# VisionDepth/VisionDepth3D

Hardware: NVIDIA H100
Metric: end-to-end frames/sec (depth+stereo) (higher is better)
Workload: dtype f16 GEMM operands, fp32 accumulate; DIBR fp32

## Files before the change

visiondepth3d_b200/csrc/umma_gemm.cuh:

```cuda
#pragma once
#include <cuda.h>
#include <cuda_fp16.h>
#include <cuda_runtime.h>
#include <stdint.h>

namespace vd3d {

enum Epi : int {
  EPI_F16 = 0,
  EPI_F32 = 1,
  EPI_RESID_LS = 2,
  EPI_QKV = 3,
  EPI_PATCH = 4,
  EPI_CONVT = 5,
  EPI_HEAD = 6,
  EPI_SR = 7,
  EPI_READOUT = 8,
};

struct GemmArgs {
  int M, N, K;
  int nt, mt, nz;
  int epi;
  int act;
  int conv;
  int cin;
  int imgW, imgH;
  int tw, th;
  __half* out_f16;
  __half* out2_f16;
  const __half* res_f16;
  float* out_f32;
  const float* bias;
  const float* ls;
  const float* pos;
  int ldc;
  long long out_batch_stride;
  __half* q;
  __half* k;
  __half* vt;
  int heads, npad, dmodel;
  float qscale;
  int ct_k, ct_cout, ct_w;
  const float* w3;
  const float* b3p;
  const __half* res2_f16;
  float rs, rs2;
  const float* img_bias;
};

namespace umma {

__device__ __forceinline__ uint32_t smem_u32(const void* p) { return (uint32_t)__cvta_generic_to_shared(p); }

__device__ __forceinline__ void mbar_init(uint32_t bar, uint32_t count) {
  asm volatile("mbarrier.init.shared::cta.b64 [%0], %1;" ::"r"(bar), "r"(count));
}
__device__ __forceinline__ void mbar_expect_tx(uint32_t bar, uint32_t bytes) {
  asm volatile("mbarrier.arrive.expect_tx.shared::cta.b64 _, [%0], %1;" ::"r"(bar), "r"(bytes) : "memory");
}
__device__ __forceinline__ void mbar_arrive(uint32_t bar) {
  asm volatile("mbarrier.arrive.shared::cta.b64 _, [%0];" ::"r"(bar) : "memory");
}
__device__ __forceinline__ void mbar_wait(uint32_t bar, uint32_t parity) {
  asm volatile(
      "{\n"
      ".reg .pred P1;\n"
      "LAB_WAIT:\n"
      "mbarrier.try_wait.parity.shared::cta.b64 P1, [%0], %1;\n"
      "@P1 bra DONE;\n"
      "bra LAB_WAIT;\n"
      "DONE:\n"
      "}\n" ::"r"(bar),
      "r"(parity)
      : "memory");
}
__device__ __forceinline__ void fence_barrier_init() {
  asm volatile("fence.mbarrier_init.release.cluster;" ::: "memory");
}

__device__ __forceinline__ void tma_load_3d(uint32_t dst, const CUtensorMap* tm, uint32_t bar, int c0, int c1,
                                            int c2) {
  asm volatile(
      "cp.async.bulk.tensor.3d.shared::cluster.global.mbarrier::complete_tx::bytes [%0], [%1, {%3, %4, %5}], [%2];"
      ::"r"(dst), "l"((uint64_t)tm), "r"(bar), "r"(c0), "r"(c1), "r"(c2)
      : "memory");
}
__device__ __forceinline__ void prefetch_tmap(const CUtensorMap* tm) {
  asm volatile("prefetch.tensormap [%0];" ::"l"((uint64_t)tm) : "memory");
}

__device__ __forceinline__ uint64_t make_desc(uint32_t smem_addr) {
  uint64_t d = 0;
  d |= (uint64_t)((smem_addr >> 4) & 0x3FFF);
  d |= (uint64_t)1 << 16;
  d |= (uint64_t)(1024 >> 4) << 32;
  d |= (uint64_t)1 << 62;
  return d;
}

__device__ __forceinline__ void wgmma_fence() { asm volatile("wgmma.fence.sync.aligned;" ::: "memory"); }
__device__ __forceinline__ void wgmma_commit() { asm volatile("wgmma.commit_group.sync.aligned;" ::: "memory"); }
template <int N>
__device__ __forceinline__ void wgmma_wait() {
  asm volatile("wgmma.wait_group.sync.aligned %0;" ::"n"(N) : "memory");
}
template <int R>
__device__ __forceinline__ void fence_regs(float (&d)[R]) {
#pragma unroll
  for (int i = 0; i < R; ++i) asm volatile("" : "+f"(d[i])::"memory");
}

#define VD3D_ACC8(i) "+f"(d[i]), "+f"(d[i + 1]), "+f"(d[i + 2]), "+f"(d[i + 3]), "+f"(d[i + 4]), "+f"(d[i + 5]), \
                     "+f"(d[i + 6]), "+f"(d[i + 7])
__device__ __forceinline__ void wgmma_m64n32_ss(float (&d)[16], uint64_t da, uint64_t db, uint32_t accumulate) {
  asm volatile(
      "{\n"
      ".reg .pred p;\n"
      "setp.ne.b32 p, %18, 0;\n"
      "wgmma.mma_async.sync.aligned.m64n32k16.f32.f16.f16 "
      "{%0, %1, %2, %3, %4, %5, %6, %7, %8, %9, %10, %11, %12, %13, %14, %15}, "
      "%16, %17, p, 1, 1, 0, 0;\n"
      "}\n"
      : VD3D_ACC8(0), VD3D_ACC8(8)
      : "l"(da), "l"(db), "r"(accumulate));
}
__device__ __forceinline__ void wgmma_m64n64_ss(float (&d)[32], uint64_t da, uint64_t db, uint32_t accumulate) {
  asm volatile(
      "{\n"
      ".reg .pred p;\n"
      "setp.ne.b32 p, %34, 0;\n"
      "wgmma.mma_async.sync.aligned.m64n64k16.f32.f16.f16 "
      "{%0, %1, %2, %3, %4, %5, %6, %7, %8, %9, %10, %11, %12, %13, %14, %15, %16, %17, %18, %19, %20, %21, %22, %23, %24, %25, %26, %27, %28, %29, %30, %31}, "
      "%32, %33, p, 1, 1, 0, 0;\n"
      "}\n"
      : VD3D_ACC8(0), VD3D_ACC8(8), VD3D_ACC8(16), VD3D_ACC8(24)
      : "l"(da), "l"(db), "r"(accumulate));
}
__device__ __forceinline__ void wgmma_m64n128_ss(float (&d)[64], uint64_t da, uint64_t db, uint32_t accumulate) {
  asm volatile(
      "{\n"
      ".reg .pred p;\n"
      "setp.ne.b32 p, %66, 0;\n"
      "wgmma.mma_async.sync.aligned.m64n128k16.f32.f16.f16 "
      "{%0, %1, %2, %3, %4, %5, %6, %7, %8, %9, %10, %11, %12, %13, %14, %15, %16, %17, %18, %19, %20, %21, %22, %23, %24, %25, %26, %27, %28, %29, %30, %31, %32, %33, %34, %35, %36, %37, %38, %39, %40, %41, %42, %43, %44, %45, %46, %47, %48, %49, %50, %51, %52, %53, %54, %55, %56, %57, %58, %59, %60, %61, %62, %63}, "
      "%64, %65, p, 1, 1, 0, 0;\n"
      "}\n"
      : VD3D_ACC8(0), VD3D_ACC8(8), VD3D_ACC8(16), VD3D_ACC8(24), VD3D_ACC8(32), VD3D_ACC8(40), VD3D_ACC8(48), VD3D_ACC8(56)
      : "l"(da), "l"(db), "r"(accumulate));
}
__device__ __forceinline__ void wgmma_m64n64_rs(float (&d)[32], const uint32_t (&a)[4], uint64_t db, uint32_t accumulate) {
  asm volatile(
      "{\n"
      ".reg .pred p;\n"
      "setp.ne.b32 p, %37, 0;\n"
      "wgmma.mma_async.sync.aligned.m64n64k16.f32.f16.f16 "
      "{%0, %1, %2, %3, %4, %5, %6, %7, %8, %9, %10, %11, %12, %13, %14, %15, %16, %17, %18, %19, %20, %21, %22, %23, %24, %25, %26, %27, %28, %29, %30, %31}, "
      "{%32, %33, %34, %35}, %36, p, 1, 1, 0;\n"
      "}\n"
      : VD3D_ACC8(0), VD3D_ACC8(8), VD3D_ACC8(16), VD3D_ACC8(24)
      : "r"(a[0]), "r"(a[1]), "r"(a[2]), "r"(a[3]), "l"(db), "r"(accumulate));
}

template <int N>
__device__ __forceinline__ void wgmma_ss(float (&d)[N / 2], uint64_t da, uint64_t db, uint32_t accumulate) {
  if constexpr (N == 32) wgmma_m64n32_ss(d, da, db, accumulate);
  else if constexpr (N == 64) wgmma_m64n64_ss(d, da, db, accumulate);
  else wgmma_m64n128_ss(d, da, db, accumulate);
}

__device__ __forceinline__ float ex2_fast(float x) {
  float y;
  asm("ex2.approx.ftz.f32 %0, %1;" : "=f"(y) : "f"(x));
  return y;
}

__device__ __forceinline__ float gelu_erf(float x) {
  const float ax = fabsf(x);
  const float z = ax * 0.70710678118654752440f;
  float t;
  asm("rcp.approx.ftz.f32 %0, %1;" : "=f"(t) : "f"(fmaf(0.3275911f, z, 1.0f)));
  float p = fmaf(t, 1.061405429f, -1.453152027f);
  p = fmaf(t, p, 1.421413741f);
  p = fmaf(t, p, -0.284496736f);
  p = fmaf(t, p, 0.254829592f);
  p *= t;
  const float e = ex2_fast(x * x * -0.72134752044448170368f);
  return fmaf(-0.5f * ax * p, e, fmaxf(x, 0.f));
}

__device__ __forceinline__ void ldg_v8(const void* p, uint32_t (&r)[8]) {
  asm volatile("ld.global.v4.b32 {%0, %1, %2, %3}, [%8];\n\t"
               "ld.global.v4.b32 {%4, %5, %6, %7}, [%8+16];"
               : "=r"(r[0]), "=r"(r[1]), "=r"(r[2]), "=r"(r[3]), "=r"(r[4]), "=r"(r[5]), "=r"(r[6]), "=r"(r[7])
               : "l"(p));
}
__device__ __forceinline__ void ldg_nc_v8(const void* p, uint32_t (&r)[8]) {
  asm volatile("ld.global.nc.v4.b32 {%0, %1, %2, %3}, [%8];\n\t"
               "ld.global.nc.v4.b32 {%4, %5, %6, %7}, [%8+16];"
               : "=r"(r[0]), "=r"(r[1]), "=r"(r[2]), "=r"(r[3]), "=r"(r[4]), "=r"(r[5]), "=r"(r[6]), "=r"(r[7])
               : "l"(p));
}
__device__ __forceinline__ void stg_v8(void* p, const uint32_t (&r)[8]) {
  asm volatile("st.global.v4.b32 [%0], {%1, %2, %3, %4};\n\t"
               "st.global.v4.b32 [%0+16], {%5, %6, %7, %8};" ::"l"(p), "r"(r[0]), "r"(r[1]), "r"(r[2]),
               "r"(r[3]), "r"(r[4]), "r"(r[5]), "r"(r[6]), "r"(r[7])
               : "memory");
}
__device__ __forceinline__ void pack16(const float (&a)[32], int base, bool relu, uint32_t (&u)[8]) {
#pragma unroll
  for (int t = 0; t < 8; ++t) {
    float x = a[base + 2 * t], y = a[base + 2 * t + 1];
    if (relu) {
      x = fmaxf(x, 0.f);
      y = fmaxf(y, 0.f);
    }
    __half2 h = __floats2half2_rn(x, y);
    u[t] = *(uint32_t*)&h;
  }
}

}

__device__ __forceinline__ void sr_epilogue_chunk(const GemmArgs& g, float (&a)[32], const int m, const int n0,
                                                  const int nvalid, const bool full) {
  if (g.out_f32) {
    float* dst = g.out_f32 + (size_t)m * g.ldc + n0;
    if (full && ((((size_t)m * g.ldc + n0) & 3) == 0)) {
#pragma unroll
      for (int j = 0; j < 8; ++j) ((float4*)dst)[j] = make_float4(a[4 * j], a[4 * j + 1], a[4 * j + 2], a[4 * j + 3]);
    } else {
#pragma unroll
      for (int j = 0; j < 32; ++j)
        if (j < nvalid) dst[j] = a[j];
    }
    return;
  }
  size_t o;
  if (g.ct_k) {
    const int tap = n0 / g.ct_cout, co = n0 % g.ct_cout;
    const int dy = tap / g.ct_k, dx = tap % g.ct_k;
    const int y = m / g.ct_w, x = m % g.ct_w;
    o = ((size_t)(y * g.ct_k + dy) * (g.ct_w * g.ct_k) + (x * g.ct_k + dx)) * g.ct_cout + co;
  } else {
    o = (size_t)m * g.ldc + n0;
  }
  const bool vec = full && ((o & 15) == 0);
#pragma unroll
  for (int q = 0; q < 2; ++q) {
    const __half* res = q == 0 ? g.res_f16 : g.res2_f16;
    if (!res) continue;
    const float sc = q == 0 ? g.rs : g.rs2;
    float rv[32];
    if (vec) {
      uint32_t u[2][8];
      umma::ldg_v8(res + o, u[0]);
      umma::ldg_v8(res + o + 16, u[1]);
#pragma unroll
      for (int j = 0; j < 2; ++j)
#pragma unroll
        for (int t = 0; t < 8; ++t) {
          const float2 f = __half22float2(*(const __half2*)&u[j][t]);
          rv[16 * j + 2 * t] = f.x;
          rv[16 * j + 2 * t + 1] = f.y;
        }
    } else {
#pragma unroll
      for (int j = 0; j < 32; ++j) rv[j] = (j < nvalid) ? __half2float(res[o + j]) : 0.f;
    }
#pragma unroll
    for (int j = 0; j < 32; ++j) a[j] = rv[j] + sc * a[j];
  }
  if (g.act == 4) {
#pragma unroll
    for (int j = 0; j < 32; ++j) a[j] = a[j] > 0.f ? a[j] : 0.2f * a[j];
  }
  if (vec) {
    uint32_t u[8];
    umma::pack16(a, 0, false, u);
    umma::stg_v8(g.out_f16 + o, u);
    umma::pack16(a, 16, false, u);
    umma::stg_v8(g.out_f16 + o + 16, u);
  } else {
#pragma unroll
    for (int j = 0; j < 32; ++j)
      if (j < nvalid) g.out_f16[o + j] = __float2half_rn(a[j]);
  }
}

template <bool kSr>
__device__ __forceinline__ void gemm_epilogue_chunk(const GemmArgs& g, const uint32_t (&v)[32], const int m, const int z,
                                                    const int n0, const bool row_ok, float& head_acc) {
  if (!row_ok || n0 >= g.N) return;
  const int nvalid = min(32, g.N - n0);
  const bool full = (nvalid == 32);
  float a[32];
  if (g.bias) {
    if (full) {
#pragma unroll
      for (int j = 0; j < 8; ++j) {
        float4 b4 = __ldg((const float4*)(g.bias + n0) + j);
        a[4 * j + 0] = __uint_as_float(v[4 * j + 0]) + b4.x;
        a[4 * j + 1] = __uint_as_float(v[4 * j + 1]) + b4.y;
        a[4 * j + 2] = __uint_as_float(v[4 * j + 2]) + b4.z;
        a[4 * j + 3] = __uint_as_float(v[4 * j + 3]) + b4.w;
      }
    } else {
#pragma unroll
      for (int j = 0; j < 32; ++j) a[j] = __uint_as_float(v[j]) + ((j < nvalid) ? g.bias[n0 + j] : 0.f);
    }
  } else {
#pragma unroll
    for (int j = 0; j < 32; ++j) a[j] = __uint_as_float(v[j]);
  }
  if constexpr (kSr) {
    sr_epilogue_chunk(g, a, m, n0, nvalid, full);
    return;
  }
  switch (g.epi) {
    case EPI_F16: {
      const size_t o = (size_t)z * g.out_batch_stride + (size_t)m * g.ldc + n0;
      const bool vec = full && ((o & 15) == 0);
      if (g.res_f16) {
        if (vec) {
          uint32_t rv[2][8];
          umma::ldg_nc_v8(g.res_f16 + o, rv[0]);
          umma::ldg_nc_v8(g.res_f16 + o + 16, rv[1]);
#pragma unroll
          for (int j = 0; j < 2; ++j)
#pragma unroll
            for (int t = 0; t < 8; ++t) {
              float2 f = __half22float2(*(const __half2*)&rv[j][t]);
              a[16 * j + 2 * t] += f.x;
              a[16 * j + 2 * t + 1] += f.y;
            }
        } else {
#pragma unroll
          for (int j = 0; j < 32; ++j)
            if (j < nvalid) a[j] += __half2float(g.res_f16[o + j]);
        }
      }
      if (g.act == 1) {
#pragma unroll
        for (int j = 0; j < 32; ++j) a[j] = umma::gelu_erf(a[j]);
      } else if (g.act == 2) {
#pragma unroll
        for (int j = 0; j < 32; ++j) a[j] = fmaxf(a[j], 0.f);
      } else if (g.act == 3) {
#pragma unroll
        for (int j = 0; j < 32; ++j)
          if (j < nvalid) a[j] = a[j] > 0.f ? a[j] : a[j] * __ldg(g.ls + n0 + j);
      }
      if (vec) {
        uint32_t u[8];
        umma::pack16(a, 0, false, u);
        umma::stg_v8(g.out_f16 + o, u);
        umma::pack16(a, 16, false, u);
        umma::stg_v8(g.out_f16 + o + 16, u);
        if (g.out2_f16) {
          umma::pack16(a, 0, true, u);
          umma::stg_v8(g.out2_f16 + o, u);
          umma::pack16(a, 16, true, u);
          umma::stg_v8(g.out2_f16 + o + 16, u);
        }
      } else {
#pragma unroll
        for (int j = 0; j < 32; ++j)
          if (j < nvalid) {
            g.out_f16[o + j] = __float2half_rn(a[j]);
            if (g.out2_f16) g.out2_f16[o + j] = __float2half_rn(fmaxf(a[j], 0.f));
          }
      }
    } break;
    case EPI_F32: {
      float* dst = g.out_f32 + (size_t)z * g.out_batch_stride + (size_t)m * g.ldc + n0;
      if (full && ((((size_t)m * g.ldc + n0) & 3) == 0) && ((g.out_batch_stride & 3) == 0)) {
#pragma unroll
        for (int j = 0; j < 8; ++j) ((float4*)dst)[j] = make_float4(a[4 * j], a[4 * j + 1], a[4 * j + 2], a[4 * j + 3]);
      } else {
#pragma unroll
        for (int j = 0; j < 32; ++j)
          if (j < nvalid) dst[j] = a[j];
      }
    } break;
    case EPI_RESID_LS: {
      float* dst = g.out_f32 + (size_t)m * g.ldc + n0;
      if (full && ((((size_t)m * g.ldc + n0) & 7) == 0)) {
        uint32_t x8[4][8];
        float4 l4[8];
#pragma unroll
        for (int j = 0; j < 4; ++j) umma::ldg_v8(dst + 8 * j, x8[j]);
#pragma unroll
        for (int j = 0; j < 8; ++j) l4[j] = __ldg((const float4*)(g.ls + n0) + j);
#pragma unroll
        for (int j = 0; j < 4; ++j) {
#pragma unroll
          for (int t = 0; t < 2; ++t) {
            const float4 l = l4[2 * j + t];
            x8[j][4 * t + 0] = __float_as_uint(fmaf(l.x, a[8 * j + 4 * t + 0], __uint_as_float(x8[j][4 * t + 0])));
            x8[j][4 * t + 1] = __float_as_uint(fmaf(l.y, a[8 * j + 4 * t + 1], __uint_as_float(x8[j][4 * t + 1])));
            x8[j][4 * t + 2] = __float_as_uint(fmaf(l.z, a[8 * j + 4 * t + 2], __uint_as_float(x8[j][4 * t + 2])));
            x8[j][4 * t + 3] = __float_as_uint(fmaf(l.w, a[8 * j + 4 * t + 3], __uint_as_float(x8[j][4 * t + 3])));
          }
        }
#pragma unroll
        for (int j = 0; j < 4; ++j) umma::stg_v8(dst + 8 * j, x8[j]);
      } else {
        float xv[32];
#pragma unroll
        for (int j = 0; j < 32; ++j) xv[j] = (j < nvalid) ? dst[j] : 0.f;
#pragma unroll
        for (int j = 0; j < 32; ++j)
          if (j < nvalid) dst[j] = xv[j] + g.ls[n0 + j] * a[j];
      }
    } break;
    case EPI_QKV: {
      const int which = n0 / g.dmodel;
      const int rem = n0 - which * g.dmodel;
      const int h = rem >> 6, d0 = rem & 63;
      const int img = m / g.npad, tok = m - img * g.npad;
      const size_t zh = (size_t)img * g.heads + h;
      if (which < 2) {
        __half* dst = (which == 0 ? g.q : g.k) + (zh * g.npad + tok) * 64 + d0;
        const float sc = which == 0 ? g.qscale : 1.0f;
#pragma unroll
        for (int j = 0; j < 32; ++j) a[j] *= sc;
        uint32_t u[8];
        umma::pack16(a, 0, false, u);
        umma::stg_v8(dst, u);
        umma::pack16(a, 16, false, u);
        umma::stg_v8(dst + 16, u);
      } else {
        __half* dst = g.vt + (zh * 64 + d0) * g.npad + tok;
#pragma unroll
        for (int j = 0; j < 32; ++j) dst[(size_t)j * g.npad] = __float2half_rn(a[j]);
      }
    } break;
    case EPI_PATCH: {
      float* dst = g.out_f32 + (size_t)(m + 1) * g.ldc + n0;
      const float* pe = g.pos + (size_t)(m + 1) * g.ldc + n0;
      float pv[32];
#pragma unroll
      for (int j = 0; j < 32; ++j) pv[j] = (j < nvalid) ? __ldg(pe + j) : 0.f;
#pragma unroll
      for (int j = 0; j < 32; ++j)
        if (j < nvalid) dst[j] = a[j] + pv[j];
    } break;
    case EPI_CONVT: {
      const int tap = n0 / g.ct_cout, co = n0 % g.ct_cout;
      const int dy = tap / g.ct_k, dx = tap % g.ct_k;
      const int y = m / g.ct_w, x = m % g.ct_w;
      size_t o = ((size_t)(y * g.ct_k + dy) * (g.ct_w * g.ct_k) + (x * g.ct_k + dx)) * g.ct_cout + co;
      if (full && ((o & 15) == 0)) {
        uint32_t u[8];
        umma::pack16(a, 0, false, u);
        umma::stg_v8(g.out_f16 + o, u);
        umma::pack16(a, 16, false, u);
        umma::stg_v8(g.out_f16 + o + 16, u);
      } else {
#pragma unroll
        for (int j = 0; j < 32; ++j)
          if (j < nvalid) g.out_f16[o + j] = __float2half_rn(a[j]);
      }
    } break;
    case EPI_HEAD: {
#pragma unroll
      for (int j = 0; j < 32; ++j)
        if (j < nvalid) head_acc += fmaxf(a[j], 0.f) * __ldg(g.w3 + n0 + j);
    } break;
    case EPI_READOUT: {
      const float* cb = g.img_bias + (size_t)(m / g.npad) * g.N + n0;
      const size_t o = (size_t)m * g.ldc + n0;
#pragma unroll
      for (int j = 0; j < 32; ++j)
        if (j < nvalid) a[j] = umma::gelu_erf(a[j] + __ldg(cb + j));
      if (full && ((o & 15) == 0)) {
        uint32_t u[8];
        umma::pack16(a, 0, false, u);
        umma::stg_v8(g.out_f16 + o, u);
        umma::pack16(a, 16, false, u);
        umma::stg_v8(g.out_f16 + o + 16, u);
      } else {
#pragma unroll
        for (int j = 0; j < 32; ++j)
          if (j < nvalid) g.out_f16[o + j] = __float2half_rn(a[j]);
      }
    } break;
  }
}

constexpr int kGemmThreads = 512;
constexpr int kBK = 64;
constexpr int kPromote = 4;
constexpr int kProducerRegs = 40;
constexpr int kEpilogueRegs = 120;
constexpr int kConsumerRegs = 176;
static_assert(128 * kProducerRegs + 128 * kEpilogueRegs + 256 * kConsumerRegs <= 65536, "register file overcommitted");

template <int BN, int STAGES>
struct GemmSmem {
  static constexpr int kABytes = 128 * kBK * 2;
  static constexpr int kBBytes = BN * kBK * 2;
  static constexpr int kStage = kABytes + kBBytes;
  static constexpr int kPitch = BN + 4;
  static constexpr int kEpi = 128 * kPitch * 4;
  static constexpr int kTotal = STAGES * kStage + kEpi + 1024  + 256 ;
};

template <int BN, int STAGES, bool kSr = false>
__global__ void __launch_bounds__(kGemmThreads, 1)
k_umma_gemm(const __grid_constant__ CUtensorMap tmA, const __grid_constant__ CUtensorMap tmB, const GemmArgs g) {
  using S = GemmSmem<BN, STAGES>;
  extern __shared__ uint8_t smem_raw[];
  uint8_t* smem = (uint8_t*)(((uintptr_t)smem_raw + 1023) & ~(uintptr_t)1023);
  float* epi_buf = (float*)(smem + STAGES * S::kStage);
  uint64_t* bars = (uint64_t*)(smem + STAGES * S::kStage + S::kEpi);
  uint64_t* full = bars;
  uint64_t* empty = bars + STAGES;
  uint64_t* epi_full = bars + 2 * STAGES;
  uint64_t* epi_empty = epi_full + 1;

  const int warp = threadIdx.x >> 5;
  const int lane = threadIdx.x & 31;
  const int total_tiles = g.nt * g.mt * g.nz;
  const int nkb = (g.K + kBK - 1) / kBK;

  if (warp == 0 && lane == 0) {
    umma::prefetch_tmap(&tmA);
    umma::prefetch_tmap(&tmB);
    for (int s = 0; s < STAGES; ++s) {
      umma::mbar_init(umma::smem_u32(&full[s]), 1);
      umma::mbar_init(umma::smem_u32(&empty[s]), 2);
    }
    umma::mbar_init(umma::smem_u32(epi_full), 256);
    umma::mbar_init(umma::smem_u32(epi_empty), 128);
    umma::fence_barrier_init();
  }
  __syncthreads();

  auto decode = [&](int tile, int& n_blk, int& m_blk, int& z, int& px0, int& py0) {
    n_blk = tile % g.nt;
    int rem = tile / g.nt;
    m_blk = rem % g.mt;
    z = rem / g.mt;
    px0 = py0 = 0;
    if (g.conv) {
      int tiles_x = (g.imgW + g.tw - 1) / g.tw;
      py0 = (m_blk / tiles_x) * g.th;
      px0 = (m_blk % tiles_x) * g.tw;
    }
  };

  if (warp < 4) {
    asm volatile("setmaxnreg.dec.sync.aligned.u32 %0;" ::"n"(kProducerRegs));
    if (warp == 0 && lane == 0) {
      int kit = 0;
      for (int tile = blockIdx.x; tile < total_tiles; tile += gridDim.x) {
        int n_blk, m_blk, z, px0, py0;
        decode(tile, n_blk, m_blk, z, px0, py0);
        for (int kb = 0; kb < nkb; ++kb, ++kit) {
          const int s = kit % STAGES;
          const uint32_t ph = (kit / STAGES) & 1;
          umma::mbar_wait(umma::smem_u32(&empty[s]), ph ^ 1);
          const uint32_t fb = umma::smem_u32(&full[s]);
          umma::mbar_expect_tx(fb, S::kStage);
          const uint32_t sa = umma::smem_u32(smem + s * S::kStage);
          const uint32_t sb = sa + S::kABytes;
          if (g.conv == 0) {
            umma::tma_load_3d(sa, &tmA, fb, kb * kBK, m_blk * 128, z);
          } else {
            const int cblocks = g.cin / kBK;
            const int tap = kb / cblocks, cb = kb % cblocks;
            int dx = 0, dy = 0;
            if (g.conv == 1) {
              dy = tap / 3 - 1;
              dx = tap % 3 - 1;
            }
            umma::tma_load_3d(sa, &tmA, fb, cb * kBK, px0 + dx, py0 + dy);
          }
          umma::tma_load_3d(sb, &tmB, fb, kb * kBK, n_blk * BN, z);
        }
      }
    }
  } else if (warp < 8) {
    asm volatile("setmaxnreg.dec.sync.aligned.u32 %0;" ::"n"(kEpilogueRegs));
    const int r = threadIdx.x & 127;
    int j = 0;
    for (int tile = blockIdx.x; tile < total_tiles; tile += gridDim.x, ++j) {
      int n_blk, m_blk, z, px0, py0;
      decode(tile, n_blk, m_blk, z, px0, py0);
      int m;
      bool row_ok;
      if (g.conv) {
        int ly = r / g.tw, lx = r % g.tw;
        int y = py0 + ly, x = px0 + lx;
        row_ok = (y < g.imgH) && (x < g.imgW);
        m = y * g.imgW + x;
      } else {
        m = m_blk * 128 + r;
        row_ok = m < g.M;
      }
      umma::mbar_wait(umma::smem_u32(epi_full), j & 1);
      float head_acc = 0.f;
#pragma unroll 1
      for (int ci = 0; ci < BN / 32; ++ci) {
        uint32_t v[32];
        const float4* src = (const float4*)(epi_buf + r * S::kPitch + ci * 32);
#pragma unroll
        for (int i = 0; i < 8; ++i) {
          const float4 f = src[i];
          v[4 * i] = __float_as_uint(f.x);
          v[4 * i + 1] = __float_as_uint(f.y);
          v[4 * i + 2] = __float_as_uint(f.z);
          v[4 * i + 3] = __float_as_uint(f.w);
        }
        gemm_epilogue_chunk<kSr>(g, v, m, z, n_blk * BN + ci * 32, row_ok, head_acc);
      }
      if (g.epi == EPI_HEAD && row_ok && n_blk == 0) g.out_f32[m] = fmaxf(head_acc + g.b3p[0], 0.f);
      umma::mbar_arrive(umma::smem_u32(epi_empty));
    }
  } else {
    asm volatile("setmaxnreg.inc.sync.aligned.u32 %0;" ::"n"(kConsumerRegs));
    const int wg = (warp >> 2) - 2;
    const int t = threadIdx.x & 127;
    const int wq = t >> 5;
    float* ebuf = epi_buf + wg * 64 * S::kPitch;
    int kit = 0;
    int j = 0;
    for (int tile = blockIdx.x; tile < total_tiles; tile += gridDim.x, ++j) {
      float acc[BN / 2];
      float tot[BN / 2];
#pragma unroll
      for (int i = 0; i < BN / 2; ++i) tot[i] = 0.f;
      int prev = -1;
      for (int kb0 = 0; kb0 < nkb; kb0 += kPromote) {
        const int kend = min(nkb, kb0 + kPromote);
        for (int kb = kb0; kb < kend; ++kb, ++kit) {
          const int s = kit % STAGES;
          const uint32_t ph = (kit / STAGES) & 1;
          umma::mbar_wait(umma::smem_u32(&full[s]), ph);
          const uint32_t sa = umma::smem_u32(smem + s * S::kStage) + (uint32_t)(wg * 64 * 128);
          const uint32_t sb = umma::smem_u32(smem + s * S::kStage) + S::kABytes;
          const uint64_t da = umma::make_desc(sa), db = umma::make_desc(sb);
          umma::wgmma_fence();
#pragma unroll
          for (int k = 0; k < kBK / 16; ++k)
            umma::wgmma_ss<BN>(acc, da + (uint64_t)(2 * k), db + (uint64_t)(2 * k), ((kb - kb0) | k) ? 1u : 0u);
          umma::wgmma_commit();
          umma::wgmma_wait<1>();
          if (prev >= 0 && t == 0) umma::mbar_arrive(umma::smem_u32(&empty[prev]));
          prev = s;
        }
        umma::wgmma_wait<0>();
        umma::fence_regs(acc);
#pragma unroll
        for (int i = 0; i < BN / 2; ++i) tot[i] += acc[i];
      }
      if (prev >= 0 && t == 0) umma::mbar_arrive(umma::smem_u32(&empty[prev]));

      umma::mbar_wait(umma::smem_u32(epi_empty), (j & 1) ^ 1);
#pragma unroll
      for (int i = 0; i < BN / 8; ++i) {
        const int c = 8 * i + 2 * (lane & 3);
        const int r0 = 16 * wq + (lane >> 2);
        *(float2*)(ebuf + r0 * S::kPitch + c) = make_float2(tot[4 * i], tot[4 * i + 1]);
        *(float2*)(ebuf + (r0 + 8) * S::kPitch + c) = make_float2(tot[4 * i + 2], tot[4 * i + 3]);
      }
      umma::mbar_arrive(umma::smem_u32(epi_full));
    }
  }
}

}
```

Before: 333.3.

## Add row-major coalesced epilogue path for aligned BN=128 GEMM tiles

Adds an epilogue mode where each warp handles whole output rows, reading the staged accumulator tile from shared memory as float4 per lane and writing 8-byte vectorised, coalesced stores across the row. Before, each thread owned one row and wrote 32 contiguous columns. The new path covers the residual, f16, QKV and readout epilogues when N, alignment and the other conditions allow. Its aim is better global-memory coalescing for the residual read-modify-write and the f16 outputs. The cost is extra code paths and per-row index arithmetic, and the V-transpose store still falls back to per-thread strided writes.

```diff
diff --git a/visiondepth3d_b200/csrc/umma_gemm.cuh b/visiondepth3d_b200/csrc/umma_gemm.cuh
--- a/visiondepth3d_b200/csrc/umma_gemm.cuh
+++ b/visiondepth3d_b200/csrc/umma_gemm.cuh
@@ -288,6 +288,13 @@
   }
 }
 
+__device__ __forceinline__ void qkv_store_vt(const GemmArgs& g, const float (&a)[32], const size_t zh, const int d0,
+                                             const int tok) {
+  __half* dst = g.vt + (zh * 64 + d0) * g.npad + tok;
+#pragma unroll
+  for (int j = 0; j < 32; ++j) dst[(size_t)j * g.npad] = __float2half_rn(a[j]);
+}
+
 template <bool kSr>
 __device__ __forceinline__ void gemm_epilogue_chunk(const GemmArgs& g, const uint32_t (&v)[32], const int m, const int z,
                                                     const int n0, const bool row_ok, float& head_acc) {
@@ -431,9 +438,7 @@
         umma::pack16(a, 16, false, u);
         umma::stg_v8(dst + 16, u);
       } else {
-        __half* dst = g.vt + (zh * 64 + d0) * g.npad + tok;
-#pragma unroll
-        for (int j = 0; j < 32; ++j) dst[(size_t)j * g.npad] = __float2half_rn(a[j]);
+        qkv_store_vt(g, a, zh, d0, tok);
       }
     } break;
     case EPI_PATCH: {
@@ -484,6 +489,186 @@
 #pragma unroll
         for (int j = 0; j < 32; ++j)
           if (j < nvalid) g.out_f16[o + j] = __float2half_rn(a[j]);
+      }
+    } break;
+  }
+}
+
+template <int BN, bool kSr>
+__device__ __forceinline__ bool gemm_launch_by_rows(const GemmArgs& g) {
+  if constexpr (BN != 128 || kSr) {
+    return false;
+  } else {
+    auto al = [](const void* p, int bytes) { return ((uintptr_t)p & (uintptr_t)(bytes - 1)) == 0; };
+    if (g.conv || (g.N & 127) || !al(g.bias, 16)) return false;
+    switch (g.epi) {
+      case EPI_RESID_LS: return (g.ldc & 3) == 0 && al(g.out_f32, 16) && al(g.ls, 16);
+      case EPI_F16:
+        return (g.ldc & 3) == 0 && (g.out_batch_stride & 3) == 0 && al(g.out_f16, 8) && al(g.out2_f16, 8) &&
+               al(g.res_f16, 8) && (g.act != 3 || al(g.ls, 16));
+      case EPI_QKV: return (g.dmodel & 127) == 0 && al(g.q, 8) && al(g.k, 8);
+      case EPI_READOUT: return (g.ldc & 3) == 0 && al(g.out_f16, 8) && al(g.img_bias, 16);
+      default: return false;
+    }
+  }
+}
+
+constexpr int kEpiRows = 4;
+
+namespace umma {
+__device__ __forceinline__ uint2 pack4(const float4 a) {
+  __half2 lo = __floats2half2_rn(a.x, a.y), hi = __floats2half2_rn(a.z, a.w);
+  return make_uint2(*(uint32_t*)&lo, *(uint32_t*)&hi);
+}
+__device__ __forceinline__ float4 lds_f4(const uint32_t addr) {
+  float4 v;
+  asm volatile("ld.shared.v4.f32 {%0, %1, %2, %3}, [%4];" : "=f"(v.x), "=f"(v.y), "=f"(v.z), "=f"(v.w) : "r"(addr));
+  return v;
+}
+__device__ __forceinline__ float4 relu4(const float4 a) {
+  return make_float4(fmaxf(a.x, 0.f), fmaxf(a.y, 0.f), fmaxf(a.z, 0.f), fmaxf(a.w, 0.f));
+}
+}
+
+__device__ __forceinline__ void gemm_epilogue_rows(const GemmArgs& g, const float* tile, const int pitch,
+                                                   const int m_blk, const int n_blk, const int z) {
+  const int w = (threadIdx.x >> 5) & 3, lane = threadIdx.x & 31;
+  const int n = n_blk * 128 + 4 * lane;
+  const int nrows = min(128, g.M - m_blk * 128);
+  const size_t row0 = (size_t)m_blk * 128;
+  const uint32_t srow = umma::smem_u32(tile) + 16 * lane;
+  const float4 b4 = g.bias ? __ldg((const float4*)(g.bias + n)) : make_float4(0.f, 0.f, 0.f, 0.f);
+  auto row_acc = [&](const int r) {
+    float4 a = umma::lds_f4(srow + r * pitch * 4);
+    if (g.bias) {
+      a.x += b4.x;
+      a.y += b4.y;
+      a.z += b4.z;
+      a.w += b4.w;
+    }
+    return a;
+  };
+  switch (g.epi) {
+    case EPI_RESID_LS: {
+      const float4 l4 = __ldg((const float4*)(g.ls + n));
+      float* const x0 = g.out_f32 + n;
+#pragma unroll 1
+      for (int r0 = w; r0 < nrows; r0 += 4 * kEpiRows) {
+        float4 x[kEpiRows];
+#pragma unroll
+        for (int i = 0; i < kEpiRows; ++i)
+          if (r0 + 4 * i < nrows) x[i] = *(const float4*)(x0 + (row0 + r0 + 4 * i) * g.ldc);
+#pragma unroll
+        for (int i = 0; i < kEpiRows; ++i) {
+          if (r0 + 4 * i >= nrows) break;
+          const float4 a = row_acc(r0 + 4 * i);
+          x[i].x = fmaf(l4.x, a.x, x[i].x);
+          x[i].y = fmaf(l4.y, a.y, x[i].y);
+          x[i].z = fmaf(l4.z, a.z, x[i].z);
+          x[i].w = fmaf(l4.w, a.w, x[i].w);
+          *(float4*)(x0 + (row0 + r0 + 4 * i) * g.ldc) = x[i];
+        }
+      }
+    } break;
+    case EPI_F16: {
+      const float4 s4 = g.act == 3 ? __ldg((const float4*)(g.ls + n)) : make_float4(0.f, 0.f, 0.f, 0.f);
+      const size_t o0 = (size_t)z * g.out_batch_stride + n;
+#pragma unroll 1
+      for (int r0 = w; r0 < nrows; r0 += 4 * kEpiRows) {
+        uint2 rv[kEpiRows];
+        if (g.res_f16) {
+#pragma unroll
+          for (int i = 0; i < kEpiRows; ++i)
+            if (r0 + 4 * i < nrows) rv[i] = __ldg((const uint2*)(g.res_f16 + o0 + (row0 + r0 + 4 * i) * g.ldc));
+        }
+#pragma unroll
+        for (int i = 0; i < kEpiRows; ++i) {
+          if (r0 + 4 * i >= nrows) break;
+          const size_t o = o0 + (row0 + r0 + 4 * i) * g.ldc;
+          float4 a = row_acc(r0 + 4 * i);
+          if (g.res_f16) {
+            const float2 f0 = __half22float2(*(const __half2*)&rv[i].x), f1 = __half22float2(*(const __half2*)&rv[i].y);
+            a.x += f0.x;
+            a.y += f0.y;
+            a.z += f1.x;
+            a.w += f1.y;
+          }
+          if (g.act == 1) {
+            a = make_float4(umma::gelu_erf(a.x), umma::gelu_erf(a.y), umma::gelu_erf(a.z), umma::gelu_erf(a.w));
+          } else if (g.act == 2) {
+            a = umma::relu4(a);
+          } else if (g.act == 3) {
+            a.x = a.x > 0.f ? a.x : a.x * s4.x;
+            a.y = a.y > 0.f ? a.y : a.y * s4.y;
+            a.z = a.z > 0.f ? a.z : a.z * s4.z;
+            a.w = a.w > 0.f ? a.w : a.w * s4.w;
+          }
+          *(uint2*)(g.out_f16 + o) = umma::pack4(a);
+          if (g.out2_f16) *(uint2*)(g.out2_f16 + o) = umma::pack4(umma::relu4(a));
+        }
+      }
+    } break;
+    case EPI_QKV: {
+      const int which = n_blk * 128 / g.dmodel;
+      if (which == 2) {
+        const int r = threadIdx.x & 127;
+        if (r >= nrows) break;
+        const int m = m_blk * 128 + r, img = m / g.npad, tok = m - img * g.npad;
+#pragma unroll 1
+        for (int ci = 0; ci < 4; ++ci) {
+          const int n0 = n_blk * 128 + 32 * ci;
+          float a[32];
+#pragma unroll
+          for (int i = 0; i < 8; ++i) {
+            float4 f = umma::lds_f4(umma::smem_u32(tile + r * pitch + 32 * ci + 4 * i));
+            if (g.bias) {
+              const float4 bb = __ldg((const float4*)(g.bias + n0) + i);
+              f.x += bb.x;
+              f.y += bb.y;
+              f.z += bb.z;
+              f.w += bb.w;
+            }
+            a[4 * i] = f.x;
+            a[4 * i + 1] = f.y;
+            a[4 * i + 2] = f.z;
+            a[4 * i + 3] = f.w;
+          }
+          const int rem = n0 - 2 * g.dmodel;
+          qkv_store_vt(g, a, (size_t)img * g.heads + (rem >> 6), rem & 63, tok);
+        }
+        break;
+      }
+      const int h = (n_blk * 128 - which * g.dmodel + 4 * lane) >> 6, d0 = (4 * lane) & 63;
+      __half* const base = which == 0 ? g.q : g.k;
+      const float sc = which == 0 ? g.qscale : 1.0f;
+#pragma unroll 4
+      for (int r = w; r < nrows; r += 4) {
+        const int m = m_blk * 128 + r;
+        const int img = m / g.npad, tok = m - img * g.npad;
+        float4 a = row_acc(r);
+        a.x *= sc;
+        a.y *= sc;
+        a.z *= sc;
+        a.w *= sc;
+        *(uint2*)(base + (((size_t)img * g.heads + h) * g.npad + tok) * 64 + d0) = umma::pack4(a);
+      }
+    } break;
+    case EPI_READOUT: {
+#pragma unroll 1
+      for (int r0 = w; r0 < nrows; r0 += 4 * kEpiRows) {
+        float4 cb[kEpiRows];
+#pragma unroll
+        for (int i = 0; i < kEpiRows; ++i)
+          if (r0 + 4 * i < nrows)
+            cb[i] = __ldg((const float4*)(g.img_bias + (size_t)((m_blk * 128 + r0 + 4 * i) / g.npad) * g.N + n));
+#pragma unroll
+        for (int i = 0; i < kEpiRows; ++i) {
+          if (r0 + 4 * i >= nrows) break;
+          const float4 a = row_acc(r0 + 4 * i);
+          const float4 y = make_float4(umma::gelu_erf(a.x + cb[i].x), umma::gelu_erf(a.y + cb[i].y),
+                                       umma::gelu_erf(a.z + cb[i].z), umma::gelu_erf(a.w + cb[i].w));
+          *(uint2*)(g.out_f16 + (row0 + r0 + 4 * i) * g.ldc + n) = umma::pack4(y);
+        }
       }
     } break;
   }
@@ -584,6 +769,17 @@
     }
   } else if (warp < 8) {
     asm volatile("setmaxnreg.dec.sync.aligned.u32 %0;" ::"n"(kEpilogueRegs));
+    if (gemm_launch_by_rows<BN, kSr>(g)) {
+      int j = 0;
+      for (int tile = blockIdx.x; tile < total_tiles; tile += gridDim.x, ++j) {
+        int n_blk, m_blk, z, px0, py0;
+        decode(tile, n_blk, m_blk, z, px0, py0);
+        umma::mbar_wait(umma::smem_u32(epi_full), j & 1);
+        gemm_epilogue_rows(g, epi_buf, S::kPitch, m_blk, n_blk, z);
+        umma::mbar_arrive(umma::smem_u32(epi_empty));
+      }
+      return;
+    }
     const int r = threadIdx.x & 127;
     int j = 0;
     for (int tile = blockIdx.x; tile < total_tiles; tile += gridDim.x, ++j) {
```

Result: faster. 360.1 (median of 6 runs) (+8.0%).
